# ka9q/ka9q-radio

Measured on NVIDIA H100. Metric: input Msamples/s through forward+filter+inverse at N channels, higher is better.
Workload: dtype f32

## Files before the change

### include/ka9q_gpu.h

```cpp
#ifndef KA9Q_GPU_H
#define KA9Q_GPU_H 1
#include <stddef.h>
#include <stdint.h>

#ifdef __cplusplus
extern "C" {
#endif

enum kgpu_type { KGPU_COMPLEX = 1, KGPU_REAL = 2 };
enum kgpu_format {
  KGPU_FMT_F32 = 0,
  KGPU_FMT_I16 = 1
};
enum kgpu_chan_flags {
  KGPU_CHAN_ISB = 1,
  KGPU_CHAN_BEAM = 4
};

typedef struct kgpu_master kgpu_master;
typedef struct kgpu_bank kgpu_bank;

struct kgpu_ingest_stats {
  unsigned long long energy;
  unsigned int clips;
// ... 118 lines not shown
int kgpu_bank_set_filter_on(kgpu_bank *b, int idx, double low, double high, double kaiser_beta, void *stream);
int kgpu_bank_set_response(kgpu_bank *b, int idx, float const *response);
int kgpu_bank_get_response(kgpu_bank *b, int idx, float *response);
int kgpu_bank_set_shift(kgpu_bank *b, int idx, int shift);
int kgpu_bank_set_flags(kgpu_bank *b, int idx, int flags);
int kgpu_bank_enable(kgpu_bank *b, int idx, int enabled);
int kgpu_bank_set_weights(kgpu_bank *b, int idx, double alpha_re, double alpha_im, double beta_re, double beta_im);
int kgpu_bank_set_osc(kgpu_bank *b, int idx, int enable, double phase_cycles, double freq_cps, double rate_cps2,
                      double block_adj_cycles);
int kgpu_bank_get_osc_phase(kgpu_bank *b, int idx, double *phase_cycles);
int kgpu_bank_set_block_counter(kgpu_bank *b, long counter);
long kgpu_bank_block_counter(kgpu_bank const *b);
int kgpu_bank_channels(kgpu_bank const *b);
long kgpu_bank_out_stride(kgpu_bank const *b);
long kgpu_bank_out_offset(kgpu_bank const *b, int idx);
int kgpu_bank_run(kgpu_bank *b, const void *d_spec, int nblocks, void *d_out, void *stream);
int kgpu_bank_run_ex(kgpu_bank *b, const void *d_spec, int nblocks, void *d_out, long out_pitch, float *d_power, void *stream);
int kgpu_bank_run_one(kgpu_bank *b, int idx, const void *d_spec, void *d_out, void *stream);
int kgpu_bank_run_one_ex(kgpu_bank *b, int idx, const void *d_spec, void *d_out, float *d_power , void *stream);
int kgpu_bank_noise(kgpu_bank *b, const void *d_spec, int nblocks, double samprate, double *d_n0, void *stream);

int kgpu_bank_fm_front(kgpu_bank *b, const void *d_out, long out_pitch, int nblocks, float *d_baseband, double *d_stats, void *stream);

int kgpu_bank_commit(kgpu_bank *b, void *stream);
int kgpu_use_static_kernels(int on);
int kgpu_use_cols_tma(int on);
int kgpu_cols_tma_fits(int L, int M, int in_type, int fmt, const void *d_in);
int kgpu_use_fused_forward(int on);
int kgpu_fused_forward_fits(int L, int M, int in_type, int fmt, const void *d_in);
int kgpu_fused_forward_options(int lead, int discard);
int kgpu_fused_shape(int *out);
int kgpu_fused_schedule(int nblocks, int lead, int ticket, int *out);
long kgpu_fused_discards(int blk, int idx, long *lines, long max);

int kgpu_plan_radices(int len, int *radices, int max);
int kgpu_plan_split(long n, int *n1, int *n2);
int kgpu_plan_radices_ex(int len, int *radices, int max);
int kgpu_plan_split_ex(long n, int *n1, int *n2);

int kgpu_multicast_copy(const void *d_src, void *mc_dst, unsigned long long bytes, int nctas, void *stream);

typedef struct kgpu_spectrum kgpu_spectrum;
kgpu_spectrum *kgpu_spectrum_create(int fft_n, int in_type, int bin_count);
int kgpu_spectrum_set_window(kgpu_spectrum *s, float const *window);
int kgpu_spectrum_run(kgpu_spectrum *s, const void *d_ring, long ring_samples, long end, int fmt, float scale,
                      const struct kgpu_scale_change *d_chg, int nchg, long long end_index, int derandomize, int shift, int fft_avg, double overlap, float *d_bins, void *stream);
int kgpu_spectrum_run_narrow(kgpu_spectrum *s, const void *d_ring, long ring_size, long ring_idx, int fft_avg,
                             double overlap, float *d_bins, int *fft_avg_used, void *stream);
int kgpu_spectrum_ring_append(void *d_ring, long ring_size, long ring_idx, const void *d_src, long olen, void *stream);
int kgpu_spectrum_describe(kgpu_spectrum const *s, char *buf, int buflen);
void kgpu_spectrum_destroy(kgpu_spectrum *s);
int kgpu_spectrum_plan(int fft_n, int in_type, char *buf, int buflen);

double kgpu_algorithmic_bytes(kgpu_master const *m, kgpu_bank const *b, int fmt);

#ifdef __cplusplus
}
#endif
#endif
```

### ka9q_radio_b200/capi.py

```python
from __future__ import annotations

import ctypes as C
import os
import subprocess
from pathlib import Path

PKG = Path(__file__).resolve().parent
LIB_PATH = PKG / "libka9qgpu.so"

KGPU_COMPLEX, KGPU_REAL = 1, 2
KGPU_FMT_F32, KGPU_FMT_I16 = 0, 1
KGPU_RAW_U8, KGPU_RAW_S8 = 1, 2
KGPU_RAW_S16, KGPU_RAW_U16, KGPU_RAW_SC16Q11 = 3, 4, 5
KGPU_RAW_F32, KGPU_RAW_CF32, KGPU_RAW_CF32_CNRMF, KGPU_RAW_CF32_FSCALE = 6, 7, 8, 9
KGPU_CHAN_ISB = 1
KGPU_CHAN_BEAM = 4

_lib = None


class KgpuError(RuntimeError):
    pass


# ... 63 lines not shown
    L.kgpu_siggen_destroy.argtypes = [vp]
    L.kgpu_siggen_generate.argtypes = [vp, ll, l, d, vp, i, vp, vp, i, l, l, vp]
    L.kgpu_siggen_state.argtypes = [vp, C.c_ulonglong, vp]
    L.kgpu_siggen_angles.argtypes = [vp, vp]
    L.filter_siggen_setup.argtypes = [vp, vp]
    L.write_genfilter.argtypes = [vp, i, d]
    L.filter_siggen_stats.argtypes = [vp, vp]
    L.kgpu_bank_define_ex.argtypes = [vp, i, i, i]
    L.kgpu_bank_define_wide.argtypes = [vp, i, i, i]
    L.kgpu_bank_define_huge.argtypes = [vp, i, i, i]
    L.kgpu_bank_define_ext.argtypes = [vp, i, i, i]
    L.kgpu_bank_define_any.argtypes = [vp, i, i, i]
    L.kgpu_chan_plan.argtypes = [i, i, C.c_char_p, i]
    L.kgpu_bank_set_weights.argtypes = [vp, i, d, d, d, d]
    L.kgpu_bank_set_osc.argtypes = [vp, i, i, d, d, d, d]
    L.kgpu_bank_get_osc_phase.argtypes = [vp, i, vp]
    L.kgpu_bank_set_block_counter.argtypes = [vp, l]
    L.kgpu_bank_block_counter.argtypes = [vp]
    L.kgpu_bank_block_counter.restype = l
    L.kgpu_bank_run_ex.argtypes = [vp, vp, i, vp, l, vp, vp]
    L.kgpu_bank_run_one_ex.argtypes = [vp, i, vp, vp, vp, vp]
    L.kgpu_bank_noise.argtypes = [vp, vp, i, d, vp, vp]
    L.kgpu_bank_fm_front.argtypes = [vp, vp, l, i, vp, vp, vp]
    L.kgpu_use_static_kernels.argtypes = [i]
    L.kgpu_use_cols_tma.argtypes = [i]
    L.kgpu_cols_tma_fits.argtypes = [i, i, i, i, vp]
    L.kgpu_use_fused_forward.argtypes = [i]
    L.kgpu_fused_forward_fits.argtypes = [i, i, i, i, vp]
    L.kgpu_fused_forward_options.argtypes = [i, i]
    L.kgpu_fused_shape.argtypes = [vp]
    L.kgpu_fused_schedule.argtypes = [i, i, i, vp]
    L.kgpu_fused_discards.argtypes = [i, i, vp, l]
    L.kgpu_fused_discards.restype = l
    L.kgpu_profile_enable.argtypes = [i]
    L.kgpu_profile_name.argtypes = [i]
    L.kgpu_profile_name.restype = C.c_char_p
    L.kgpu_profile_get.argtypes = [i, vp, vp]
    L.kgpu_plan_radices.argtypes = [i, vp, i]
    L.kgpu_plan_split.argtypes = [l, vp, vp]
    L.kgpu_plan_radices_ex.argtypes = [i, vp, i]
    L.kgpu_plan_split_ex.argtypes = [l, vp, vp]
    L.kgpu_multicast_copy.argtypes = [vp, vp, C.c_ulonglong, i, vp]
    L.kgpu_algorithmic_bytes.argtypes = [vp, vp, i]
    L.kgpu_algorithmic_bytes.restype = d
    L.kgpu_spectrum_create.restype = vp
    L.kgpu_spectrum_create.argtypes = [i, i, i]
    L.kgpu_spectrum_set_window.argtypes = [vp, vp]
    L.kgpu_spectrum_run.argtypes = [vp, vp, l, l, i, f, vp, i, C.c_longlong, i, i, i, d, vp, vp]
    L.kgpu_spectrum_run_narrow.argtypes = [vp, vp, l, l, i, d, vp, vp, vp]
    L.kgpu_spectrum_ring_append.argtypes = [vp, l, l, vp, l, vp]
    L.kgpu_spectrum_describe.argtypes = [vp, C.c_char_p, i]
    L.kgpu_spectrum_destroy.argtypes = [vp]
    L.kgpu_spectrum_plan.argtypes = [i, i, C.c_char_p, i]
    _lib = L
    return L


def exported_symbols() -> list[str]:
    import re

    hdr = (PKG.parent / "include" / "ka9q_gpu.h").read_text()
    hdr = re.sub(r"/\*.*?\*/", " ", hdr, flags=re.S)
    return sorted(set(re.findall(r"\b(kgpu_[a-z0-9_]+)\s*\(", hdr)))


def profile_snapshot() -> dict[str, tuple[float, int]]:
# ... 351 lines not shown
```

### ka9q_radio_b200/csrc/fwd_cols_r36.cuh

```cuda
#pragma once
#include <cuda.h>

#include "static_kernels_v2.cuh"

namespace kfft {

struct ColsR36Tables {
  float2 const *tw0;
  float2 const *twA;
  float2 const *twB;
};

__device__ __forceinline__ float2 r36_power(float2 const (&wb)[6], float2 const (&wa)[6], int t) {
  int const a = t / 6, b = t - 6 * a;
  if (a == 0) return wb[b];
  if (b == 0) return wa[a];
  return cmul(wa[a], wb[b]);
}

struct ColsR36Shape {
  static constexpr int BLK = 38, CP = 1378, T = 288;
  static constexpr size_t smem = sizeof(float2) * (size_t)(8 * CP + 360 + 80);
};

struct ColsR36Tma {
  static constexpr int BOX_ROWS = 216;
  static constexpr int F32_BOX_BYTES = BOX_ROWS * 64;
  static constexpr int I16_BOX_WORDS = 12, I16_BOX_BYTES = BOX_ROWS * I16_BOX_WORDS * 4;
  static constexpr int I16_ODD_OFF = 3 * I16_BOX_BYTES;
  static constexpr uint32_t bytes(int fmt) { return fmt == 0 ? 6 * F32_BOX_BYTES : 6 * I16_BOX_BYTES; }
};
static_assert(ColsR36Tma::bytes(0) + 112 <= sizeof(float2) * 8 * ColsR36Shape::CP &&
              ColsR36Tma::bytes(1) + 112 <= sizeof(float2) * 8 * ColsR36Shape::CP, "the raw tile lies in the float tile");
static_assert(ColsR36Tma::F32_BOX_BYTES % 128 == 0 && ColsR36Tma::I16_BOX_BYTES % 128 == 0, "box destinations 128-B aligned");

template <int FMT>
__device__ __forceinline__ float2 r36_ingest(int raw, int row, int col, int n2, Pass1Args const &a, unsigned long long &energy,
                                             unsigned int &clips) {
  int lo, hi;
  unpack_i16(raw, lo, hi);
  if (FMT == 2) {
    if (a.derandomize) {
      lo ^= (lo & 1) ? 0xfffffffe : 0;
      hi ^= (hi & 1) ? 0xfffffffe : 0;
    }
    if (a.stats && (long)row * n2 + col >= a.first_new) {
      energy += (unsigned long long)(lo * lo) + (unsigned long long)(hi * hi);
      clips += (lo > 32766 || lo < -32766) + (hi > 32766 || hi < -32766);
    }
  }
  return make_float2(i32_to_f32(lo), i32_to_f32(hi));
}

__device__ __forceinline__ void r36_stage0_store(float2 (&x)[36], float2 const *s_tw0, float2 *d, int ul) {
  constexpr int R = 36, BLK = ColsR36Shape::BLK;
  float2 wb[6], wa[6];
#pragma unroll
  for (int b = 1; b < 6; b++) {
    wb[b] = s_tw0[(b - 1) * 36 + ul];
    wa[b] = s_tw0[(4 + b) * 36 + ul];
  }
  d[0] = x[0];
#pragma unroll
  for (int t = 1; t < R; t++) d[t * BLK] = cmul(x[t], r36_power(wb, wa, t));
}

template <int FMT, int N2C, bool TMA, class Sync>
__device__ __forceinline__ void fwd_cols_r36_body(Pass1Args const &a, ColsR36Tables const &tb, CUtensorMap const *tmap,
                                                  unsigned char *smem_raw, uint64_t &tbar, int tid, int c0, int blk,
                                                  Sync const &sync) {
  constexpr int R = 36, BLK = ColsR36Shape::BLK, CP = ColsR36Shape::CP;
  float2 *tile = reinterpret_cast<float2 *>(smem_raw);
  float2 *s_tw0 = tile + 8 * CP;
  float2 *s_twB = s_tw0 + 360;
  int const c = tid & 7, ul = tid >> 3;
  int const n2 = N2C ? N2C : a.n2;
  int const ld = N2C ? (N2C + 15) / 16 * 16 : a.mid_ld;
  int const ncols = min(8, n2 - c0);
  bool const col_ok = c < ncols;
  int const n2g = c0 + c;
  float2 *mycol = tile + c * CP;
  unsigned char *const rtile = smem_raw + ((0u - smem_u32(smem_raw)) & 127u);
  if (tid == 0) {
    mbar_init(&tbar, 1);
    mbar_fence_init();
    if constexpr (TMA) {
      using T = ColsR36Tma;
      mbar_expect_tx(&tbar, 360 * 8 + 80 * 8 + T::bytes(FMT));
      if (FMT == 0) {
#pragma unroll
        for (int k = 0; k < 6; k++) tensor_g2s_3d(rtile + k * T::F32_BOX_BYTES, tmap, 2 * c0, k * T::BOX_ROWS, blk, &tbar);
      } else {
#pragma unroll
        for (int k = 0; k < 3; k++) {
          tensor_g2s_3d(rtile + k * T::I16_BOX_BYTES, tmap, c0, k * T::BOX_ROWS, blk, &tbar);
          tensor_g2s_3d(rtile + T::I16_ODD_OFF + k * T::I16_BOX_BYTES, tmap, n2 + c0 - (n2 & 2), k * T::BOX_ROWS, blk, &tbar);
        }
      }
    } else {
      mbar_expect_tx(&tbar, 360 * 8 + 80 * 8);
    }
    bulk_g2s(s_tw0, tb.tw0, 360 * 8, &tbar);
    bulk_g2s(s_twB, tb.twB + (long)c0 * 10, 80 * 8, &tbar);
  }
  sync();
  float2 const twA = col_ok ? ldg_stream_f2(tb.twA + (long)n2g * 36 + ul) : make_float2(1.f, 0.f);

  unsigned long long energy = 0;
  unsigned int clips = 0;
  if constexpr (TMA) {
    float2 x[R];
    mbar_wait(&tbar, 0);
    if (col_ok) {
      if (FMT == 0) {
        float2 const *src = reinterpret_cast<float2 const *>(rtile) + ul * 8 + c;
#pragma unroll
        for (int m = 0; m < R; m++) x[m] = src[R * 8 * m];
      } else {
        using T = ColsR36Tma;
        int const odd = ul & 1;
        int const *src = reinterpret_cast<int const *>(rtile + odd * T::I16_ODD_OFF) + (ul >> 1) * T::I16_BOX_WORDS + c +
                         odd * (n2 & 2);
#pragma unroll
        for (int m = 0; m < R; m++)
          x[m] = r36_ingest<FMT>(src[(R / 2) * T::I16_BOX_WORDS * m], ul + R * m, n2g, n2, a, energy, clips);
      }
      Dft<R, false>::run(x);
    }
    sync();
    if (col_ok) r36_stage0_store(x, s_tw0, mycol + ul, ul);
  } else if (col_ok) {
    float2 x[R];
    if (FMT == 0) {
      float2 const *src = reinterpret_cast<float2 const *>(a.in) + (long)blk * a.hop + n2g + (long)ul * n2;
#pragma unroll
      for (int m = 0; m < R; m++) x[m] = ldg_stream_f2(src + (long)(R * m) * n2);
    } else {
      int const *src = reinterpret_cast<int const *>(a.in) + (long)blk * a.hop + n2g + (long)ul * n2;
      int raw[R];
#pragma unroll
      for (int m = 0; m < R; m++) raw[m] = ldg_stream_b32(src + (long)(R * m) * n2);
#pragma unroll
      for (int m = 0; m < R; m++) x[m] = r36_ingest<FMT>(raw[m], ul + R * m, n2g, n2, a, energy, clips);
    }
    mbar_wait(&tbar, 0);
    Dft<R, false>::run(x);
    r36_stage0_store(x, s_tw0, mycol + ul, ul);
  } else {
    mbar_wait(&tbar, 0);
  }
  if (FMT == 2 && a.stats) {
#pragma unroll
    for (int o = 16; o > 0; o >>= 1) {
      energy += __shfl_xor_sync(0xffffffffu, energy, o);
      clips += __shfl_xor_sync(0xffffffffu, clips, o);
    }
    if ((tid & 31) == 0 && (energy | clips)) {
      atomicAdd(&a.stats[blk].energy, energy);
      atomicAdd(&a.stats[blk].clips, clips);
    }
  }
  sync();

  if (col_ok) {
    float2 x[R];
    float4 const *p4 = reinterpret_cast<float4 const *>(mycol + ul * BLK);
#pragma unroll
    for (int m = 0; m < R / 2; m++) {
      float4 const v = p4[m];
      x[2 * m] = make_float2(v.x, v.y);
      x[2 * m + 1] = make_float2(v.z, v.w);
    }
    Dft<R, false>::run(x);
    float2 wb[6], wa[6];
#pragma unroll
    for (int b = 1; b < 6; b++) {
      wb[b] = s_twB[c * 10 + (b - 1)];
      wa[b] = s_twB[c * 10 + (4 + b)];
    }
    float2 const w0 = make_float2(twA.x * a.out_scale, twA.y * a.out_scale);
    float2 *dst = a.mid + (long)blk * 1296 * ld + n2g + (long)ul * ld;
    dst[0] = cmul(x[0], w0);
#pragma unroll
    for (int k = 1; k < R; k++) dst[(long)(R * k) * ld] = cmul(x[k], cmul(w0, r36_power(wb, wa, k)));
  }
}

template <int FMT, int N2C>
__global__ void __launch_bounds__(ColsR36Shape::T, 2) fwd_cols_r36(Pass1Args const a, ColsR36Tables const tb) {
  extern __shared__ __align__(16) unsigned char smem_raw[];
  __shared__ __align__(8) uint64_t tbar;
  fwd_cols_r36_body<FMT, N2C, false>(a, tb, nullptr, smem_raw, tbar, threadIdx.x, blockIdx.x * 8, blockIdx.y,
                                     [] { __syncthreads(); });
}
template <int FMT, int N2C>
__global__ void __launch_bounds__(ColsR36Shape::T, 2)
    fwd_cols_r36_tma(Pass1Args const a, ColsR36Tables const tb, const __grid_constant__ CUtensorMap tmap) {
  extern __shared__ __align__(16) unsigned char smem_raw[];
  __shared__ __align__(8) uint64_t tbar;
  fwd_cols_r36_body<FMT, N2C, true>(a, tb, &tmap, smem_raw, tbar, threadIdx.x, blockIdx.x * 8, blockIdx.y,
                                    [] { __syncthreads(); });
}

}
```

### ka9q_radio_b200/csrc/fwd_fused.cuh

```cuda
#pragma once
#include "fwd_cols_r36.cuh"
#include "static_kernels_v2.cuh"

namespace kfft {

struct FusedShape {
  static constexpr int N1 = 1296, N2 = 1250;
  static constexpr int TILES = (N2 + 7) / 8;
  static constexpr int NC = (TILES + 1) / 2;
  static constexpr int NR = (N1 / 2 + 1 + RowsV2Shape<true>::IPC - 1) / RowsV2Shape<true>::IPC;
  static constexpr int T = 2 * ColsR36Shape::T;
  static constexpr int RT = RowsV2Shape<true>::T;
  static constexpr size_t smem = 2 * ColsR36Shape::smem > RowsV2Shape<true>::smem ? 2 * ColsR36Shape::smem : RowsV2Shape<true>::smem;
  static constexpr int DEFAULT_LEAD = 40;
  static_assert(ColsR36Shape::smem % 16 == 0, "the second tile's memory 16-byte aligned");
  static_assert(T % 32 == 0 && ColsR36Shape::T % 32 == 0 && RT % 32 == 0, "whole warps per tile and per R item");
};

enum FusedKind : int { kFusedCol = 0, kFusedRow = 1 };
struct FusedItem {
  int kind, blk, idx;
};

__host__ __device__ __forceinline__ FusedItem fused_item(int t, int nblocks, int lead) {
// ... 9 lines not shown
}

struct FusedArgs {
  unsigned *ctr;
  int nblocks, lead;
  int discard;
};

__device__ __forceinline__ void red_release_gpu_add(unsigned *p, unsigned v) {
  asm volatile("red.release.gpu.global.add.u32 [%0], %1;" ::"l"(p), "r"(v) : "memory");
}
__device__ __forceinline__ unsigned ld_acquire_gpu(unsigned const *p) {
  unsigned v;
  asm volatile("ld.acquire.gpu.global.u32 %0, [%1];" : "=r"(v) : "l"(p) : "memory");
  return v;
}

template <int FMT>
__global__ void __launch_bounds__(FusedShape::T, 1)
    fwd_fused_r36_v2(Pass1Args const a1, ColsR36Tables const t1, Pass2Args const a2, FwdTables const t2, FusedArgs const f,
                     const __grid_constant__ CUtensorMap tmap) {
  using F = FusedShape;
  extern __shared__ __align__(16) unsigned char smem_raw[];
  __shared__ __align__(8) uint64_t bars[RowsV2Shape<true>::COLS];
  __shared__ __align__(8) uint64_t tbar[2];
  __shared__ int s_ticket;
  int const tid = threadIdx.x;
  if (tid == 0) s_ticket = (int)atomicAdd(f.ctr, 1u);
  __syncthreads();
  FusedItem const it = fused_item(s_ticket, f.nblocks, f.lead);
  if (it.kind == kFusedCol) {
    int const h = tid >= ColsR36Shape::T, tile = 2 * it.idx + h;
    if (tile < F::TILES)
      fwd_cols_r36_body<FMT, F::N2, true>(a1, t1, &tmap, smem_raw + h * ColsR36Shape::smem, tbar[h], tid - h * ColsR36Shape::T,
                                           tile * 8, it.blk, [h] {
                                             asm volatile("bar.sync %0, %1;" ::"r"(1 + h), "n"(ColsR36Shape::T) : "memory");
                                           });
    __syncthreads();
    if (tid == 0) {
      __threadfence();
      red_release_gpu_add(f.ctr + 1 + fused_item(s_ticket, f.nblocks, f.lead).blk, 1u);
    }
    return;
  }
  if (tid >= F::RT) return;
  auto sync = [] { asm volatile("bar.sync 3, %0;" ::"n"(F::RT) : "memory"); };
  auto sync_or = [](int p) {
    int r;
    asm volatile("{\n\t.reg .pred q, o;\n\tsetp.ne.s32 q, %1, 0;\n\tbar.red.or.pred o, 3, %2, q;\n\tselp.s32 %0, 1, 0, o;\n\t}"
                 : "=r"(r)
                 : "r"(p), "n"(F::RT)
                 : "memory");
    return r;
  };
  if (tid == 0)
    while (ld_acquire_gpu(f.ctr + 1 + it.blk) < (unsigned)F::NC) __nanosleep(64);
  sync();
  fwd_rows_v2_body<true, F::N1, true, true>(a2, t2, smem_raw, bars, tbar[0], tid, it.blk, it.idx * RowsV2Shape<true>::IPC,
                                            sync, sync_or, f.discard);
}

}
```

### ka9q_radio_b200/csrc/kgpu.cu

```cuda
#include <cuda_runtime.h>
#include <cudaTypedefs.h>
#include <math.h>
#include <stdarg.h>
#include <stdio.h>
#include <stdlib.h>
#include <string.h>
#include <algorithm>
#include <complex>
#include <atomic>
#include <map>
#include <mutex>
#include <string>
#include <vector>

#include "../../include/ka9q_gpu.h"
#include "chan_kernels.cuh"
#include "chan_huge.cuh"
#include "chan_wide.cuh"
#include "fwd_kernels.cuh"
#include "noise_kernel.cuh"
#include "plan.cuh"
#include "static_kernels.cuh"
#include "static_kernels_v2.cuh"
#include "fwd_cols_r36.cuh"
#include "fwd_fused.cuh"
#include "fwd_2s.cuh"
#include "spectrum_kernels.cuh"
#include "bluestein_master.cuh"
#include "bluestein_chan.cuh"
#include "raw_ingest.cuh"
#include "iq_correct.cuh"
#include "siggen.cuh"

using namespace kfft;

static thread_local std::string g_err;
static std::atomic<unsigned long long> g_launches{0};

static std::atomic<int> g_static_on{1};
extern "C" int kgpu_use_static_kernels(int on) {
  g_static_on.store(on != 0);
  return 0;
}
static std::atomic<int> g_cols_tma{-1};
extern "C" int kgpu_use_cols_tma(int on) {
  g_cols_tma.store(on != 0);
  return 0;
}
static bool cols_tma_on() {
  int v = g_cols_tma.load();
  if (v < 0) {
    char const *e = getenv("KA9Q_COLS_TMA");
    g_cols_tma.compare_exchange_strong(v, (e && *e) ? (atoi(e) != 0) : 1);
    v = g_cols_tma.load();
  }
  return v != 0;
}
static std::atomic<int> g_fused{-1};
static std::atomic<int> g_fused_lead{FusedShape::DEFAULT_LEAD}, g_fused_discard{0};
extern "C" int kgpu_use_fused_forward(int on) {
  g_fused.store(on != 0);
  return 0;
}
static bool fused_on() {
  int v = g_fused.load();
  if (v < 0) {
    char const *e = getenv("KA9Q_FUSED_FWD");
    g_fused.compare_exchange_strong(v, (e && *e) ? (atoi(e) != 0) : 1);
    v = g_fused.load();
  }
  return v != 0;
}

static int fail(char const *fmt, ...) {
  char buf[512];
  va_list ap;
  va_start(ap, fmt);
  vsnprintf(buf, sizeof buf, fmt, ap);
  va_end(ap);
  g_err = buf;
  return -1;
}
#define CUDA_OK(expr)                                                                    \
  do {                                                                                   \
    cudaError_t e_ = (expr);                                                             \
    if (e_ != cudaSuccess) return fail("%s: %s (%s:%d)", #expr, cudaGetErrorString(e_), __FILE__, __LINE__); \
  } while (0)
#define CUDA_OKP(expr)                                                                   \
  do {                                                                                   \
    cudaError_t e_ = (expr);                                                             \
    if (e_ != cudaSuccess) {                                                             \
      fail("%s: %s (%s:%d)", #expr, cudaGetErrorString(e_), __FILE__, __LINE__);         \
      return nullptr;                                                                    \
    }                                                                                    \
  } while (0)

static int allow_smem(const void *func, size_t bytes) {
  if (bytes <= 48 * 1024) return 0;
  static std::mutex mu;
  static std::map<std::pair<int, const void *>, size_t> granted;
  int dev = 0;
  CUDA_OK(cudaGetDevice(&dev));
  std::lock_guard<std::mutex> lk(mu);
  size_t &g = granted[{dev, func}];
// ... 885 lines not shown
using ColsR36Fn = void (*)(Pass1Args, ColsR36Tables);
using ColsR36TmaFn = void (*)(Pass1Args, ColsR36Tables, CUtensorMap);
using Cols2sFn = void (*)(Pass1Args, Cols2sTables);
using RowsV2Fn = void (*)(Pass2Args, FwdTables);
using Cols2s = Cols2sShape<25, 32>;
using Rows2s = Rows2sShape<25, 25>;
static ColsR36Fn cols_r36_kernel(kgpu_master const *m, int f) {
  static ColsR36Fn const k[2][3] = {{fwd_cols_r36<0, 0>, fwd_cols_r36<1, 0>, fwd_cols_r36<2, 0>},
                                    {fwd_cols_r36<0, 1250>, fwd_cols_r36<1, 1250>, fwd_cols_r36<2, 1250>}};
  return k[m->n2c == 1250][f];
}
static ColsR36TmaFn cols_r36_tma_kernel(kgpu_master const *m, int f) {
  static ColsR36TmaFn const k[2][3] = {{fwd_cols_r36_tma<0, 0>, fwd_cols_r36_tma<1, 0>, fwd_cols_r36_tma<2, 0>},
                                       {fwd_cols_r36_tma<0, 1250>, fwd_cols_r36_tma<1, 1250>, fwd_cols_r36_tma<2, 1250>}};
  return k[m->n2c == 1250][f];
}
static Cols2sFn cols_2s_kernel(int f) {
  static Cols2sFn const k[3] = {fwd_cols_2s<0, 25, 32>, fwd_cols_2s<1, 25, 32>, fwd_cols_2s<2, 25, 32>};
  return k[f];
}
static RowsV2Fn rows_v2_kernel(kgpu_master const *m) {
  if (m->in_type == KGPU_REAL) return m->halved ? fwd_rows_v2<true, 1296, true> : fwd_rows_v2<true, 0, false>;
  return m->n1c ? fwd_rows_v2<false, 1296, false> : fwd_rows_v2<false, 0, false>;
}
static bool fused_pair(kgpu_master const *m) {
  return m->in_type == KGPU_REAL && m->cols == COLS_R36 && m->rows == ROWS_V2 && m->halved && m->n2c == FusedShape::N2 &&
         m->n1c == FusedShape::N1 && m->mid_ld % 16 == 0;
}
using FusedFn = void (*)(Pass1Args, ColsR36Tables, Pass2Args, FwdTables, FusedArgs, CUtensorMap);
static FusedFn fused_kernel(int f) {
  static FusedFn const k[3] = {fwd_fused_r36_v2<0>, fwd_fused_r36_v2<1>, fwd_fused_r36_v2<2>};
  return k[f];
}
static int rows_v2_threads(kgpu_master const *m) { return m->in_type == KGPU_REAL ? RowsV2Shape<true>::T : RowsV2Shape<false>::T; }
static size_t rows_v2_smem(kgpu_master const *m) {
  return m->in_type == KGPU_REAL ? RowsV2Shape<true>::smem : RowsV2Shape<false>::smem;
}

static int upload(float2 **d, std::vector<float2> const &v) {
  CUDA_OK(cudaMalloc(d, sizeof(float2) * v.size()));
  CUDA_OK(cudaMemcpy(*d, v.data(), sizeof(float2) * v.size(), cudaMemcpyHostToDevice));
  return 0;
}

static int bluestein_upload(Bluestein *b) {
  if (upload(&b->d_b, bluestein_bspec(b->n, b->P)) == 0) return 0;
  cudaFree(b->d_b);
  b->d_b = nullptr;
  return -1;
}

static void master_geometry(kgpu_master *m, int L, int M, int in_type) {
  m->L = L;
  m->M = M;
  m->N = L + M - 1;
  m->in_type = in_type;
  m->bins = (in_type == KGPU_COMPLEX) ? m->N : m->N / 2 + 1;
  m->nc = (in_type == KGPU_COMPLEX) ? m->N : m->N / 2;
  m->spec_stride = ((long)m->bins + 3) / 4 * 4;
}

static void master_shape(kgpu_master *m, int L, int M, int in_type, Split2 const &sp, bool ext) {
  master_geometry(m, L, M, in_type);
  m->sp = sp;
  m->ext = ext;
  m->pitch1 = column_pitch(sp.n1);
// ... 48 lines not shown
    std::vector<float2> t0(360), tA((size_t)n2 * 36), tB((size_t)(n2 + 8) * 10, make_float2(0.f, 0.f));
    for (int e = 0; e < 10; e++)
      for (int j = 0; j < 36; j++) t0[(size_t)e * 36 + j] = root((long)j * kPow[e], 1296);
    for (long c = 0; c < n2; c++) {
      for (int t = 0; t < 36; t++) tA[(size_t)c * 36 + t] = root(c * t, m->nc);
      for (int e = 0; e < 10; e++) tB[(size_t)c * 10 + e] = root(c * 36 * kPow[e], m->nc);
    }
    if (upload(&m->d_tw0, t0) || upload(&m->d_twA, tA) || upload(&m->d_twB, tB)) return -1;
    for (int f = 0; f < 3; f++)
      if (allow_smem((const void *)cols_r36_kernel(m, f), ColsR36Shape::smem) ||
          allow_smem((const void *)cols_r36_tma_kernel(m, f), ColsR36Shape::smem))
        return -1;
  }
  if (m->cols == COLS_2S) {
    constexpr int RA = 25, RB = 32, RC = 25, RD = 25;
    std::vector<float2> t0((size_t)Cols2s::TW0, make_float2(0.f, 0.f)), tA((size_t)n2 * RA),
        tB((size_t)(n2 + 8) * Cols2s::NP1, make_float2(0.f, 0.f)), r0((size_t)Rows2s::TW0, make_float2(0.f, 0.f));
    for (int e = 0; e < Cols2s::NP0; e++)
      for (int j = 0; j < RB; j++) t0[(size_t)e * RB + j] = root((long)j * Pow<RA>::exponent(e), n1);
    for (long c = 0; c < n2; c++) {
      for (int t = 0; t < RA; t++) tA[(size_t)c * RA + t] = root(c * t, m->nc);
      for (int e = 0; e < Cols2s::NP1; e++) tB[(size_t)c * Cols2s::NP1 + e] = root(c * RA * Pow<RB>::exponent(e), m->nc);
    }
    for (int e = 0; e < Rows2s::NP0; e++)
      for (int j = 0; j < RD; j++) r0[(size_t)e * RD + j] = root((long)j * Pow<RC>::exponent(e), n2);
    if (upload(&m->d_tw0, t0) || upload(&m->d_twA, tA) || upload(&m->d_twB, tB) || upload(&m->d_rtw0, r0)) return -1;
    for (int f = 0; f < 3; f++)
      if (allow_smem((const void *)cols_2s_kernel(f), Cols2s::smem)) return -1;
    if (allow_smem((const void *)fwd_rows_2s<25, 25>, Rows2s::smem)) return -1;
  }
  if (m->rows == ROWS_V2 && allow_smem((const void *)rows_v2_kernel(m), rows_v2_smem(m))) return -1;
  if (fused_pair(m))
    for (int f = 0; f < 3; f++)
      if (allow_smem((const void *)fused_kernel(f), FusedShape::smem)) return -1;
  if (m->ext) {
    if (allow_smem((const void *)fwd_cols_ext<0>, m->smem1) || allow_smem((const void *)fwd_cols_ext<1>, m->smem1) ||
        allow_smem((const void *)fwd_rows_ext, m->smem2))
      return -1;
  } else if (allow_smem((const void *)fwd_cols_kernel<0>, m->smem1) || allow_smem((const void *)fwd_cols_kernel<1>, m->smem1) ||
             allow_smem((const void *)fwd_rows_kernel, m->smem2)) {
    return -1;
  }
  return 0;
}

extern "C" void kgpu_master_destroy(kgpu_master *m) {
  if (!m) return;
  if (m->ext) {
    free_tile_plan(m->xplan1);
    free_tile_plan(m->xplan2);
  }
  cudaFree(m->d_rootD);
  cudaFree(m->d_rootC);
  cudaFree(m->d_tw0);
  cudaFree(m->d_twA);
  cudaFree(m->d_twB);
  cudaFree(m->d_rtw0);
  cudaFree(m->mid.p);
  cudaFree(m->fused_ctr.p);
  cudaFree(m->d_notch);
  kgpu_master_destroy(m->bs);
  cudaFree(m->blue.d_b);
  cudaFree(m->b_in.p);
  cudaFree(m->b_out.p);
  delete m;
}
extern "C" int kgpu_master_points(kgpu_master const *m) { return m ? m->N : -1; }
// ... 180 lines not shown
  return fused_fits(&m, d_in, fmt) ? 1 : 0;
}

extern "C" int kgpu_fused_forward_options(int lead, int discard) {
  if (lead < 0 || lead > FusedShape::NC) return fail("kgpu_fused_forward_options: lead %d outside 0..%d", lead, FusedShape::NC);
  g_fused_lead.store(lead);
  g_fused_discard.store(discard != 0);
  return 0;
}

extern "C" int kgpu_fused_shape(int *out) {
  if (!out) return fail("kgpu_fused_shape: bad arguments");
  out[0] = FusedShape::NC;
  out[1] = FusedShape::NR;
  out[2] = FusedShape::N1;
  out[3] = (FusedShape::N2 + 15) / 16 * 16;
  out[4] = FusedShape::DEFAULT_LEAD;
  return 0;
}

extern "C" int kgpu_fused_schedule(int nblocks, int lead, int ticket, int *out) {
  if (nblocks < 1 || lead < 0 || lead > FusedShape::NC || ticket < 0 || ticket >= nblocks * (FusedShape::NC + FusedShape::NR) ||
      !out)
    return fail("kgpu_fused_schedule: bad arguments");
  FusedItem const it = fused_item(ticket, nblocks, lead);
  out[0] = it.kind;
  out[1] = it.blk;
  out[2] = it.idx;
  out[3] = it.kind == kFusedRow ? it.blk : -1;
  out[4] = it.kind == kFusedRow ? FusedShape::NC : 0;
  return 0;
}

extern "C" long kgpu_fused_discards(int blk, int idx, long *lines, long max) {
  using S = RowsV2Shape<true>;
  if (blk < 0 || idx < 0 || idx >= FusedShape::NR || max < 0) return fail("kgpu_fused_discards: bad arguments");
  int const ld = (FusedShape::N2 + 15) / 16 * 16;
  long n = 0;
  for (int col = 0; col < S::COLS; col++) {
    RowItem const it = row_item(idx * S::IPC + (col >> 1), FusedShape::N1, true);
    int const row = (col & 1) == 0 ? (it.kind != kRowEmpty ? it.row_a : -1) : (it.kind == kRowPair ? it.row_b : -1);
    if (row < 0) continue;
    for (int l = 0; l < mid_row_lines(ld); l++, n++)
      if (lines && n < max) lines[n] = mid_line(blk, FusedShape::N1, row, ld, l);
  }
  return n;
}

static int cols_tma_map(kgpu_master const *m, void const *d_in, int fmt, int nblocks, CUtensorMap *map) {
  static PFN_cuTensorMapEncodeTiled const encode = [] {
    void *fn = nullptr;
    cudaDriverEntryPointQueryResult q;
    if (cudaGetDriverEntryPoint("cuTensorMapEncodeTiled", &fn, cudaEnableDefault, &q) != cudaSuccess ||
        q != cudaDriverEntryPointSuccess)
      fn = nullptr;
    return (PFN_cuTensorMapEncodeTiled)fn;
  }();
  if (!encode) return fail("kgpu_forward: the driver has no cuTensorMapEncodeTiled");
  bool const i16 = fmt == KGPU_FMT_I16;
  cuuint64_t const n1 = (cuuint64_t)m->sp.n1, n2 = (cuuint64_t)m->sp.n2;
  cuuint64_t const hop = (cuuint64_t)(m->in_type == KGPU_REAL ? m->L / 2 : m->L);
  cuuint64_t const dim[3] = {2 * n2, i16 ? n1 / 2 : n1, (cuuint64_t)nblocks};
  cuuint64_t const stride[2] = {8 * n2, hop * (i16 ? 4 : 8)};
  cuuint32_t const box[3] = {(cuuint32_t)(i16 ? ColsR36Tma::I16_BOX_WORDS : 16), ColsR36Tma::BOX_ROWS, 1};
  cuuint32_t const unit[3] = {1, 1, 1};
  CUresult const r = encode(map, i16 ? CU_TENSOR_MAP_DATA_TYPE_UINT32 : CU_TENSOR_MAP_DATA_TYPE_FLOAT32, 3, const_cast<void *>(d_in),
                            dim, stride, box, unit, CU_TENSOR_MAP_INTERLEAVE_NONE, CU_TENSOR_MAP_SWIZZLE_NONE,
                            CU_TENSOR_MAP_L2_PROMOTION_L2_128B, CU_TENSOR_MAP_FLOAT_OOB_FILL_NONE);
  if (r != CUDA_SUCCESS) return fail("kgpu_forward: cuTensorMapEncodeTiled failed (%d)", (int)r);
  return 0;
}

static Pass2Args rows_args(kgpu_master const *m, Pass1Args const &a1, void *d_spec) {
  Pass2Args a2;
  a2.mid = a1.mid;
  a2.n1 = m->sp.n1;
  a2.n2 = m->sp.n2;
  a2.nc = m->nc;
  a2.plan = m->plan2;
  a2.pitch = m->pitch2;
  a2.real_split = (m->in_type == KGPU_REAL);
  a2.rootD = m->d_rootD;
  a2.spec = (float2 *)d_spec;
  a2.spec_stride = m->spec_stride;
  a2.mid_ld = a1.mid_ld;
  return a2;
}

static int fused_span(kgpu_master *m, const void *d_in, int fmt, int f, int nblocks, void *d_spec, cudaStream_t st,
                      Pass1Args const &a1) {
  using F = FusedShape;
  size_t const ctr_bytes = sizeof(unsigned) * (size_t)(1 + nblocks);
  if (grow(m->fused_ctr, ctr_bytes, st, "kgpu_forward")) return -1;
  CUtensorMap map;
  if (cols_tma_map(m, d_in, fmt, nblocks, &map)) return -1;
  FusedArgs fa;
  fa.ctr = (unsigned *)m->fused_ctr.p;
  fa.nblocks = nblocks;
  fa.lead = g_fused_lead.load();
  fa.discard = g_fused_discard.load();
  CUDA_OK(cudaMemsetAsync(fa.ctr, 0, ctr_bytes, st));
  {
    ProfScope ps(K_FWD_FUSED, st);
    fused_kernel(f)<<<(unsigned)(nblocks * (F::NC + F::NR)), F::T, F::smem, st>>>(a1, ColsR36Tables{m->d_tw0, m->d_twA, m->d_twB},
                                                                       rows_args(m, a1, d_spec), FwdTables{m->d_rootC}, fa, map);
  }
  g_launches++;
  CUDA_OK(cudaGetLastError());
  return 0;
}

static int forward_span(kgpu_master *m, const void *d_in, int fmt, float scale, int derandomize, int nblocks, void *d_spec,
                        void *d_stats, cudaStream_t st, float2 *mid) {
  bool const use_static = g_static_on.load() != 0;
  ColsKernel const cols = use_static ? m->cols : COLS_GENERIC;
  RowsKernel const rows = use_static ? m->rows : ROWS_GENERIC;
  Pass1Args a1;
  a1.in = d_in;
  a1.hop = (m->in_type == KGPU_REAL) ? m->L / 2 : m->L;
  a1.n1 = m->sp.n1;
  a1.n2 = m->sp.n2;
  a1.nc = m->nc;
  a1.plan = m->plan1;
  a1.pitch = m->pitch1;
  a1.scale = scale;
  a1.derandomize = derandomize;
  a1.first_new = (m->in_type == KGPU_REAL) ? (m->M - 1) / 2 : (m->M - 1);
  a1.mid = mid;
  a1.stats = (fmt == KGPU_FMT_I16) ? (IngestStats *)d_stats : nullptr;
  a1.out_scale = (fmt == KGPU_FMT_I16 ? scale : 1.0f) * (m->halved ? 0.5f : 1.0f);
  a1.mid_ld = use_static ? m->mid_ld : m->sp.n2;
  int const f = (fmt != KGPU_FMT_I16) ? 0 : ((derandomize || a1.stats) ? 2 : 1);
  if (nblocks >= 2 && use_static && cols_tma_on() && fused_on() && fused_fits(m, d_in, fmt)) return fused_span(m, d_in, fmt, f, nblocks, d_spec, st, a1);
  dim3 const g1((unsigned)((m->sp.n2 + kTile - 1) / kTile), (unsigned)nblocks);
  {
    ProfScope ps(K_FWD_COLS, st);
    switch (cols) {
      case COLS_2S:
        cols_2s_kernel(f)<<<g1, Cols2s::T, Cols2s::smem, st>>>(a1, Cols2sTables{m->d_tw0, m->d_twA, m->d_twB});
        break;
      case COLS_R36:
        if (cols_tma_on() && cols_tma_fits(m, d_in, fmt)) {
          CUtensorMap map;
          if (cols_tma_map(m, d_in, fmt, nblocks, &map)) return -1;
          cols_r36_tma_kernel(m, f)<<<g1, ColsR36Shape::T, ColsR36Shape::smem, st>>>(a1, ColsR36Tables{m->d_tw0, m->d_twA, m->d_twB}, map);
        } else {
          cols_r36_kernel(m, f)<<<g1, ColsR36Shape::T, ColsR36Shape::smem, st>>>(a1, ColsR36Tables{m->d_tw0, m->d_twA, m->d_twB});
        }
        break;
      case COLS_GENERIC:
        if (m->ext && f) fwd_cols_ext<1><<<g1, kFwdThreads, m->smem1, st>>>(a1, m->xplan1);
        else if (m->ext) fwd_cols_ext<0><<<g1, kFwdThreads, m->smem1, st>>>(a1, m->xplan1);
        else if (f) fwd_cols_kernel<1><<<g1, kFwdThreads, m->smem1, st>>>(a1);
        else fwd_cols_kernel<0><<<g1, kFwdThreads, m->smem1, st>>>(a1);
        break;
    }
  }
  g_launches++;
  Pass2Args const a2 = rows_args(m, a1, d_spec);
  dim3 const g2((unsigned)(rows == ROWS_GENERIC ? m->n_item_ctas : m->n_rows_ctas), (unsigned)nblocks);
  {
    ProfScope ps(K_FWD_ROWS, st);
    switch (rows) {
      case ROWS_2S:
        fwd_rows_2s<25, 25><<<g2, Rows2s::T, Rows2s::smem, st>>>(a2, m->d_rtw0);
        break;
// ... 1353 lines not shown
```

Measured before the change: 103,600.

## Add persistent warp-specialized fused forward kernel and L2 evict-last mid stores

Adds an opt-in persistent fused forward kernel (mode 3) that splits each CTA into a row-pass engine and a 4-column column-pass engine. The two engines pull work tickets from global counters and synchronize per block through release/acquire counters. The column tile geometry is templated on column count. Separately, the existing fused kernel now writes the intermediate mid buffer with an L2 evict_last cache hint so the rows pass can re-read it from L2. The new kernel runs only via env/setting, and the hint may displace other L2 data.

```diff
diff --git a/include/ka9q_gpu.h b/include/ka9q_gpu.h
--- a/include/ka9q_gpu.h
+++ b/include/ka9q_gpu.h
@@ -174,6 +174,8 @@
 int kgpu_fused_shape(int *out);
 int kgpu_fused_schedule(int nblocks, int lead, int ticket, int *out);
 long kgpu_fused_discards(int blk, int idx, long *lines, long max);
+int kgpu_fused2_shape(int *out);
+int kgpu_fused2_schedule(int nblocks, int queue, int ticket, int *out);
 
 int kgpu_plan_radices(int len, int *radices, int max);
 int kgpu_plan_split(long n, int *n1, int *n2);
diff --git a/ka9q_radio_b200/capi.py b/ka9q_radio_b200/capi.py
--- a/ka9q_radio_b200/capi.py
+++ b/ka9q_radio_b200/capi.py
@@ -119,6 +119,8 @@
     L.kgpu_fused_schedule.argtypes = [i, i, i, vp]
     L.kgpu_fused_discards.argtypes = [i, i, vp, l]
     L.kgpu_fused_discards.restype = l
+    L.kgpu_fused2_shape.argtypes = [vp]
+    L.kgpu_fused2_schedule.argtypes = [i, i, i, vp]
     L.kgpu_profile_enable.argtypes = [i]
     L.kgpu_profile_name.argtypes = [i]
     L.kgpu_profile_name.restype = C.c_char_p
diff --git a/ka9q_radio_b200/csrc/fwd_cols_r36.cuh b/ka9q_radio_b200/csrc/fwd_cols_r36.cuh
--- a/ka9q_radio_b200/csrc/fwd_cols_r36.cuh
+++ b/ka9q_radio_b200/csrc/fwd_cols_r36.cuh
@@ -18,21 +18,28 @@
   return cmul(wa[a], wb[b]);
 }
 
-struct ColsR36Shape {
-  static constexpr int BLK = 38, CP = 1378, T = 288;
-  static constexpr size_t smem = sizeof(float2) * (size_t)(8 * CP + 360 + 80);
+template <int NCOL>
+struct ColsR36Geom {
+  static_assert(NCOL == 8 || NCOL == 4, "8- or 4-column tiles");
+  static constexpr int BLK = 38, CP = NCOL == 8 ? 1378 : 1380, T = (36 * NCOL + 31) / 32 * 32;
+  static constexpr int LOG = NCOL == 8 ? 3 : 2;
+  static constexpr size_t smem = sizeof(float2) * (size_t)(NCOL * CP + 360 + 10 * NCOL);
 };
-
-struct ColsR36Tma {
+using ColsR36Shape = ColsR36Geom<8>;
+
+template <int NCOL>
+struct ColsR36TmaT {
   static constexpr int BOX_ROWS = 216;
-  static constexpr int F32_BOX_BYTES = BOX_ROWS * 64;
-  static constexpr int I16_BOX_WORDS = 12, I16_BOX_BYTES = BOX_ROWS * I16_BOX_WORDS * 4;
+  static constexpr int F32_BOX_FLOATS = 2 * NCOL, F32_BOX_BYTES = BOX_ROWS * F32_BOX_FLOATS * 4;
+  static constexpr int I16_BOX_WORDS = NCOL + 4, I16_BOX_BYTES = BOX_ROWS * I16_BOX_WORDS * 4;
   static constexpr int I16_ODD_OFF = 3 * I16_BOX_BYTES;
   static constexpr uint32_t bytes(int fmt) { return fmt == 0 ? 6 * F32_BOX_BYTES : 6 * I16_BOX_BYTES; }
+  static_assert(bytes(0) + 112 <= sizeof(float2) * NCOL * ColsR36Geom<NCOL>::CP &&
+                bytes(1) + 112 <= sizeof(float2) * NCOL * ColsR36Geom<NCOL>::CP, "the raw tile lies in the float tile");
+  static_assert(F32_BOX_BYTES % 128 == 0 && I16_BOX_BYTES % 128 == 0, "box destinations 128-B aligned");
+  static_assert(F32_BOX_FLOATS * 4 % 16 == 0 && I16_BOX_WORDS * 4 % 16 == 0, "box widths whole 16-byte units");
 };
-static_assert(ColsR36Tma::bytes(0) + 112 <= sizeof(float2) * 8 * ColsR36Shape::CP &&
-              ColsR36Tma::bytes(1) + 112 <= sizeof(float2) * 8 * ColsR36Shape::CP, "the raw tile lies in the float tile");
-static_assert(ColsR36Tma::F32_BOX_BYTES % 128 == 0 && ColsR36Tma::I16_BOX_BYTES % 128 == 0, "box destinations 128-B aligned");
+using ColsR36Tma = ColsR36TmaT<8>;
 
 template <int FMT>
 __device__ __forceinline__ float2 r36_ingest(int raw, int row, int col, int n2, Pass1Args const &a, unsigned long long &energy,
@@ -65,19 +72,20 @@
   for (int t = 1; t < R; t++) d[t * BLK] = cmul(x[t], r36_power(wb, wa, t));
 }
 
-template <int FMT, int N2C, bool TMA, class Sync>
+template <int FMT, int N2C, bool TMA, int NCOL = 8, bool KEEP_MID = false, class Sync>
 __device__ __forceinline__ void fwd_cols_r36_body(Pass1Args const &a, ColsR36Tables const &tb, CUtensorMap const *tmap,
                                                   unsigned char *smem_raw, uint64_t &tbar, int tid, int c0, int blk,
                                                   Sync const &sync) {
-  constexpr int R = 36, BLK = ColsR36Shape::BLK, CP = ColsR36Shape::CP;
+  using G = ColsR36Geom<NCOL>;
+  constexpr int R = 36, BLK = G::BLK, CP = G::CP;
   float2 *tile = reinterpret_cast<float2 *>(smem_raw);
-  float2 *s_tw0 = tile + 8 * CP;
+  float2 *s_tw0 = tile + NCOL * CP;
   float2 *s_twB = s_tw0 + 360;
-  int const c = tid & 7, ul = tid >> 3;
+  int const c = tid & (NCOL - 1), ul = tid >> G::LOG;
   int const n2 = N2C ? N2C : a.n2;
   int const ld = N2C ? (N2C + 15) / 16 * 16 : a.mid_ld;
-  int const ncols = min(8, n2 - c0);
-  bool const col_ok = c < ncols;
+  int const ncols = min(NCOL, n2 - c0);
+  bool const col_ok = c < ncols && (G::T == R * NCOL || ul < R);
   int const n2g = c0 + c;
   float2 *mycol = tile + c * CP;
   unsigned char *const rtile = smem_raw + ((0u - smem_u32(smem_raw)) & 127u);
@@ -85,8 +93,8 @@
     mbar_init(&tbar, 1);
     mbar_fence_init();
     if constexpr (TMA) {
-      using T = ColsR36Tma;
-      mbar_expect_tx(&tbar, 360 * 8 + 80 * 8 + T::bytes(FMT));
+      using T = ColsR36TmaT<NCOL>;
+      mbar_expect_tx(&tbar, 360 * 8 + NCOL * 80 + T::bytes(FMT));
       if (FMT == 0) {
 #pragma unroll
         for (int k = 0; k < 6; k++) tensor_g2s_3d(rtile + k * T::F32_BOX_BYTES, tmap, 2 * c0, k * T::BOX_ROWS, blk, &tbar);
@@ -98,10 +106,10 @@
         }
       }
     } else {
-      mbar_expect_tx(&tbar, 360 * 8 + 80 * 8);
+      mbar_expect_tx(&tbar, 360 * 8 + NCOL * 80);
     }
     bulk_g2s(s_tw0, tb.tw0, 360 * 8, &tbar);
-    bulk_g2s(s_twB, tb.twB + (long)c0 * 10, 80 * 8, &tbar);
+    bulk_g2s(s_twB, tb.twB + (long)c0 * 10, NCOL * 80, &tbar);
   }
   sync();
   float2 const twA = col_ok ? ldg_stream_f2(tb.twA + (long)n2g * 36 + ul) : make_float2(1.f, 0.f);
@@ -113,11 +121,11 @@
     mbar_wait(&tbar, 0);
     if (col_ok) {
       if (FMT == 0) {
-        float2 const *src = reinterpret_cast<float2 const *>(rtile) + ul * 8 + c;
-#pragma unroll
-        for (int m = 0; m < R; m++) x[m] = src[R * 8 * m];
+        float2 const *src = reinterpret_cast<float2 const *>(rtile) + ul * NCOL + c;
+#pragma unroll
+        for (int m = 0; m < R; m++) x[m] = src[R * NCOL * m];
       } else {
-        using T = ColsR36Tma;
+        using T = ColsR36TmaT<NCOL>;
         int const odd = ul & 1;
         int const *src = reinterpret_cast<int const *>(rtile + odd * T::I16_ODD_OFF) + (ul >> 1) * T::I16_BOX_WORDS + c +
                          odd * (n2 & 2);
@@ -180,9 +188,20 @@
     }
     float2 const w0 = make_float2(twA.x * a.out_scale, twA.y * a.out_scale);
     float2 *dst = a.mid + (long)blk * 1296 * ld + n2g + (long)ul * ld;
-    dst[0] = cmul(x[0], w0);
-#pragma unroll
-    for (int k = 1; k < R; k++) dst[(long)(R * k) * ld] = cmul(x[k], cmul(w0, r36_power(wb, wa, k)));
+    if constexpr (KEEP_MID) {
+      uint64_t pol;
+      asm("createpolicy.fractional.L2::evict_last.b64 %0, 1.0;" : "=l"(pol));
+      auto st = [pol](float2 *p, float2 v) {
+        asm volatile("st.global.L2::cache_hint.v2.f32 [%0], {%1, %2}, %3;" ::"l"(p), "f"(v.x), "f"(v.y), "l"(pol) : "memory");
+      };
+      st(dst, cmul(x[0], w0));
+#pragma unroll
+      for (int k = 1; k < R; k++) st(dst + (long)(R * k) * ld, cmul(x[k], cmul(w0, r36_power(wb, wa, k))));
+    } else {
+      dst[0] = cmul(x[0], w0);
+#pragma unroll
+      for (int k = 1; k < R; k++) dst[(long)(R * k) * ld] = cmul(x[k], cmul(w0, r36_power(wb, wa, k)));
+    }
   }
 }
 
diff --git a/ka9q_radio_b200/csrc/fwd_fused.cuh b/ka9q_radio_b200/csrc/fwd_fused.cuh
--- a/ka9q_radio_b200/csrc/fwd_fused.cuh
+++ b/ka9q_radio_b200/csrc/fwd_fused.cuh
@@ -65,7 +65,7 @@
   if (it.kind == kFusedCol) {
     int const h = tid >= ColsR36Shape::T, tile = 2 * it.idx + h;
     if (tile < F::TILES)
-      fwd_cols_r36_body<FMT, F::N2, true>(a1, t1, &tmap, smem_raw + h * ColsR36Shape::smem, tbar[h], tid - h * ColsR36Shape::T,
+      fwd_cols_r36_body<FMT, F::N2, true, 8, true>(a1, t1, &tmap, smem_raw + h * ColsR36Shape::smem, tbar[h], tid - h * ColsR36Shape::T,
                                            tile * 8, it.blk, [h] {
                                              asm volatile("bar.sync %0, %1;" ::"r"(1 + h), "n"(ColsR36Shape::T) : "memory");
                                            });
diff --git a/ka9q_radio_b200/csrc/fwd_fused2.cuh b/ka9q_radio_b200/csrc/fwd_fused2.cuh
--- /dev/null
+++ b/ka9q_radio_b200/csrc/fwd_fused2.cuh
@@ -0,0 +1,122 @@
+#pragma once
+#include "fwd_fused.cuh"
+
+namespace kfft {
+
+struct Fused2Shape {
+  static constexpr int N1 = 1296, N2 = 1250, NCOL = 4;
+  using CG = ColsR36Geom<NCOL>;
+  static constexpr int NT = (N2 + NCOL - 1) / NCOL;
+  static constexpr int NR = FusedShape::NR;
+  static constexpr int LAG = 2;
+  static constexpr int RT = RowsV2Shape<true>::T;
+  static constexpr int CT = CG::T;
+  static constexpr int T = RT + CT;
+  static constexpr size_t row_smem = RowsV2Shape<true>::smem;
+  static constexpr size_t smem = row_smem + CG::smem;
+  static_assert(row_smem % 16 == 0, "the column engine's memory 16-byte aligned");
+  static_assert(T % 32 == 0 && CT % 32 == 0 && RT % 32 == 0, "whole warps per engine");
+  static_assert(smem + 256 <= 227 * 1024, "both engines' shared memory in one SM");
+};
+
+enum Fused2Queue : int { kFused2Col = 0, kFused2Row = 1 };
+struct Fused2Item {
+  int blk, idx;
+  int wait, need;
+};
+__host__ __device__ __forceinline__ Fused2Item fused2_item(int queue, int t, int nblocks) {
+  using F = Fused2Shape;
+  if (queue == kFused2Col) {
+    int const b = t / F::NT;
+    return b >= F::LAG ? Fused2Item{b, t - b * F::NT, 2 + nblocks + b - F::LAG, F::NR} : Fused2Item{b, t - b * F::NT, -1, 0};
+  }
+  int const b = t / F::NR;
+  return {b, t - b * F::NR, 2 + b, F::NT};
+}
+
+struct Fused2Args {
+  unsigned *ctr;
+  int nblocks;
+};
+
+__device__ __forceinline__ void fence_proxy_async_smem() { asm volatile("fence.proxy.async.shared::cta;" ::: "memory"); }
+__device__ __forceinline__ void mbar_inval(uint64_t *bar) {
+  asm volatile("mbarrier.inval.shared::cta.b64 [%0];" ::"r"(smem_u32(bar)) : "memory");
+}
+__device__ __forceinline__ void fused2_wait(unsigned const *ctr, Fused2Item const &it) {
+  if (it.wait >= 0)
+    while (ld_acquire_gpu(ctr + it.wait) < (unsigned)it.need) __nanosleep(64);
+}
+
+template <int FMT>
+__global__ void __launch_bounds__(Fused2Shape::T, 1)
+    fwd_fused_r36_v3(Pass1Args const a1, ColsR36Tables const t1, Pass2Args const a2, FwdTables const t2, Fused2Args const f,
+                     const __grid_constant__ CUtensorMap tmap) {
+  using F = Fused2Shape;
+  extern __shared__ __align__(16) unsigned char smem_raw[];
+  __shared__ __align__(8) uint64_t bars[RowsV2Shape<true>::COLS];
+  __shared__ __align__(8) uint64_t tbar[2];
+  __shared__ int s_ticket[2];
+  int const tid = threadIdx.x;
+  if (tid < F::RT) {
+    auto sync = [] { asm volatile("bar.sync 3, %0;" ::"n"(F::RT) : "memory"); };
+    auto sync_or = [](int p) {
+      int r;
+      asm volatile("{\n\t.reg .pred q, o;\n\tsetp.ne.s32 q, %1, 0;\n\tbar.red.or.pred o, 3, %2, q;\n\tselp.s32 %0, 1, 0, o;\n\t}"
+                   : "=r"(r)
+                   : "r"(p), "n"(F::RT)
+                   : "memory");
+      return r;
+    };
+    int const total = f.nblocks * F::NR;
+    for (;;) {
+      if (tid == 0) {
+        int const t = (int)atomicAdd(f.ctr + 1, 1u);
+        s_ticket[0] = t;
+        if (t < total) fused2_wait(f.ctr, fused2_item(kFused2Row, t, f.nblocks));
+      }
+      sync();
+      int const t = s_ticket[0];
+      if (t >= total) return;
+      Fused2Item const it = fused2_item(kFused2Row, t, f.nblocks);
+      fwd_rows_v2_body<true, F::N1, true, true>(a2, t2, smem_raw, bars, tbar[0], tid, it.blk, it.idx * RowsV2Shape<true>::IPC,
+                                                sync, sync_or, false);
+      fence_proxy_async_smem();
+      sync();
+      if ((tid & 31) == 0) {
+        mbar_inval(&bars[tid >> 5]);
+        if (tid == 0) {
+          mbar_inval(&tbar[0]);
+          __threadfence();
+          red_release_gpu_add(f.ctr + 2 + f.nblocks + it.blk, 1u);
+        }
+      }
+    }
+  } else {
+    int const ct = tid - F::RT;
+    auto sync = [] { asm volatile("bar.sync 4, %0;" ::"n"(F::CT) : "memory"); };
+    unsigned char *const smem = smem_raw + F::row_smem;
+    int const total = f.nblocks * F::NT;
+    for (;;) {
+      if (ct == 0) {
+        int const t = (int)atomicAdd(f.ctr, 1u);
+        s_ticket[1] = t;
+        if (t < total) fused2_wait(f.ctr, fused2_item(kFused2Col, t, f.nblocks));
+      }
+      sync();
+      int const t = s_ticket[1];
+      if (t >= total) return;
+      Fused2Item const it = fused2_item(kFused2Col, t, f.nblocks);
+      fwd_cols_r36_body<FMT, F::N2, true, F::NCOL, true>(a1, t1, &tmap, smem, tbar[1], ct, it.idx * F::NCOL, it.blk, sync);
+      fence_proxy_async_smem();
+      sync();
+      if (ct == 0) {
+        mbar_inval(&tbar[1]);
+        __threadfence();
+        red_release_gpu_add(f.ctr + 2 + it.blk, 1u);
+      }
+    }
+  }
+}
+
+}
diff --git a/ka9q_radio_b200/csrc/kgpu.cu b/ka9q_radio_b200/csrc/kgpu.cu
--- a/ka9q_radio_b200/csrc/kgpu.cu
+++ b/ka9q_radio_b200/csrc/kgpu.cu
@@ -24,6 +24,7 @@
 #include "static_kernels_v2.cuh"
 #include "fwd_cols_r36.cuh"
 #include "fwd_fused.cuh"
+#include "fwd_fused2.cuh"
 #include "fwd_2s.cuh"
 #include "spectrum_kernels.cuh"
 #include "bluestein_master.cuh"
@@ -56,20 +57,22 @@
   }
   return v != 0;
 }
+enum FusedMode { kFusedOff = 0, kFusedDefault = 1, kFusedV2 = 2, kFusedV3 = 3 };
 static std::atomic<int> g_fused{-1};
 static std::atomic<int> g_fused_lead{FusedShape::DEFAULT_LEAD}, g_fused_discard{0};
+static int fused_mode_of(int on) { return on >= kFusedOff && on <= kFusedV3 ? on : kFusedDefault; }
 extern "C" int kgpu_use_fused_forward(int on) {
-  g_fused.store(on != 0);
-  return 0;
-}
-static bool fused_on() {
+  g_fused.store(fused_mode_of(on));
+  return 0;
+}
+static int fused_mode() {
   int v = g_fused.load();
   if (v < 0) {
     char const *e = getenv("KA9Q_FUSED_FWD");
-    g_fused.compare_exchange_strong(v, (e && *e) ? (atoi(e) != 0) : 1);
+    g_fused.compare_exchange_strong(v, (e && *e) ? fused_mode_of(atoi(e)) : kFusedDefault);
     v = g_fused.load();
   }
-  return v != 0;
+  return v == kFusedDefault ? kFusedV2 : v;
 }
 
 static int fail(char const *fmt, ...) {
@@ -1021,6 +1024,11 @@
   static FusedFn const k[3] = {fwd_fused_r36_v2<0>, fwd_fused_r36_v2<1>, fwd_fused_r36_v2<2>};
   return k[f];
 }
+using Fused2Fn = void (*)(Pass1Args, ColsR36Tables, Pass2Args, FwdTables, Fused2Args, CUtensorMap);
+static Fused2Fn fused2_kernel(int f) {
+  static Fused2Fn const k[3] = {fwd_fused_r36_v3<0>, fwd_fused_r36_v3<1>, fwd_fused_r36_v3<2>};
+  return k[f];
+}
 static int rows_v2_threads(kgpu_master const *m) { return m->in_type == KGPU_REAL ? RowsV2Shape<true>::T : RowsV2Shape<false>::T; }
 static size_t rows_v2_smem(kgpu_master const *m) {
   return m->in_type == KGPU_REAL ? RowsV2Shape<true>::smem : RowsV2Shape<false>::smem;
@@ -1135,7 +1143,8 @@
   if (m->rows == ROWS_V2 && allow_smem((const void *)rows_v2_kernel(m), rows_v2_smem(m))) return -1;
   if (fused_pair(m))
     for (int f = 0; f < 3; f++)
-      if (allow_smem((const void *)fused_kernel(f), FusedShape::smem)) return -1;
+      if (allow_smem((const void *)fused_kernel(f), FusedShape::smem) || allow_smem((const void *)fused2_kernel(f), Fused2Shape::smem))
+        return -1;
   if (m->ext) {
     if (allow_smem((const void *)fwd_cols_ext<0>, m->smem1) || allow_smem((const void *)fwd_cols_ext<1>, m->smem1) ||
         allow_smem((const void *)fwd_rows_ext, m->smem2))
@@ -1382,6 +1391,27 @@
   return 0;
 }
 
+extern "C" int kgpu_fused2_shape(int *out) {
+  if (!out) return fail("kgpu_fused2_shape: bad arguments");
+  out[0] = Fused2Shape::NT;
+  out[1] = Fused2Shape::NR;
+  out[2] = Fused2Shape::LAG;
+  out[3] = Fused2Shape::NCOL;
+  return 0;
+}
+
+extern "C" int kgpu_fused2_schedule(int nblocks, int queue, int ticket, int *out) {
+  int const per = queue == kFused2Col ? Fused2Shape::NT : Fused2Shape::NR;
+  if (nblocks < 1 || (queue != kFused2Col && queue != kFused2Row) || ticket < 0 || ticket >= nblocks * per || !out)
+    return fail("kgpu_fused2_schedule: bad arguments");
+  Fused2Item const it = fused2_item(queue, ticket, nblocks);
+  out[0] = it.blk;
+  out[1] = it.idx;
+  out[2] = it.wait;
+  out[3] = it.need;
+  return 0;
+}
+
 extern "C" long kgpu_fused_discards(int blk, int idx, long *lines, long max) {
   using S = RowsV2Shape<true>;
   if (blk < 0 || idx < 0 || idx >= FusedShape::NR || max < 0) return fail("kgpu_fused_discards: bad arguments");
@@ -1397,7 +1427,9 @@
   return n;
 }
 
+template <int NCOL = 8>
 static int cols_tma_map(kgpu_master const *m, void const *d_in, int fmt, int nblocks, CUtensorMap *map) {
+  using T = ColsR36TmaT<NCOL>;
   static PFN_cuTensorMapEncodeTiled const encode = [] {
     void *fn = nullptr;
     cudaDriverEntryPointQueryResult q;
@@ -1412,7 +1444,9 @@
   cuuint64_t const hop = (cuuint64_t)(m->in_type == KGPU_REAL ? m->L / 2 : m->L);
   cuuint64_t const dim[3] = {2 * n2, i16 ? n1 / 2 : n1, (cuuint64_t)nblocks};
   cuuint64_t const stride[2] = {8 * n2, hop * (i16 ? 4 : 8)};
-  cuuint32_t const box[3] = {(cuuint32_t)(i16 ? ColsR36Tma::I16_BOX_WORDS : 16), ColsR36Tma::BOX_ROWS, 1};
+  cuuint32_t const box[3] = {(cuuint32_t)(i16 ? T::I16_BOX_WORDS : T::F32_BOX_FLOATS), T::BOX_ROWS, 1};
+  if (NCOL * 4 % 16 != 0 || (i16 && (n2 - (n2 & 2)) % 4 != 0))
+    return fail("kgpu_forward: %d-column tensor boxes would start off 16-byte alignment", NCOL);
   cuuint32_t const unit[3] = {1, 1, 1};
   CUresult const r = encode(map, i16 ? CU_TENSOR_MAP_DATA_TYPE_UINT32 : CU_TENSOR_MAP_DATA_TYPE_FLOAT32, 3, const_cast<void *>(d_in),
                             dim, stride, box, unit, CU_TENSOR_MAP_INTERLEAVE_NONE, CU_TENSOR_MAP_SWIZZLE_NONE,
@@ -1454,6 +1488,30 @@
     ProfScope ps(K_FWD_FUSED, st);
     fused_kernel(f)<<<(unsigned)(nblocks * (F::NC + F::NR)), F::T, F::smem, st>>>(a1, ColsR36Tables{m->d_tw0, m->d_twA, m->d_twB},
                                                                        rows_args(m, a1, d_spec), FwdTables{m->d_rootC}, fa, map);
+  }
+  g_launches++;
+  CUDA_OK(cudaGetLastError());
+  return 0;
+}
+
+static int fused2_span(kgpu_master *m, const void *d_in, int fmt, int f, int nblocks, void *d_spec, cudaStream_t st,
+                       Pass1Args const &a1) {
+  using F = Fused2Shape;
+  size_t const ctr_bytes = sizeof(unsigned) * (size_t)(2 + 2 * nblocks);
+  if (grow(m->fused_ctr, ctr_bytes, st, "kgpu_forward")) return -1;
+  CUtensorMap map;
+  if (cols_tma_map<F::NCOL>(m, d_in, fmt, nblocks, &map)) return -1;
+  int dev = 0, sms = 0;
+  CUDA_OK(cudaGetDevice(&dev));
+  CUDA_OK(cudaDeviceGetAttribute(&sms, cudaDevAttrMultiProcessorCount, dev));
+  Fused2Args fa;
+  fa.ctr = (unsigned *)m->fused_ctr.p;
+  fa.nblocks = nblocks;
+  CUDA_OK(cudaMemsetAsync(fa.ctr, 0, ctr_bytes, st));
+  {
+    ProfScope ps(K_FWD_FUSED, st);
+    fused2_kernel(f)<<<(unsigned)sms, F::T, F::smem, st>>>(a1, ColsR36Tables{m->d_tw0, m->d_twA, m->d_twB}, rows_args(m, a1, d_spec),
+                                                           FwdTables{m->d_rootC}, fa, map);
   }
   g_launches++;
   CUDA_OK(cudaGetLastError());
@@ -1481,7 +1539,9 @@
   a1.out_scale = (fmt == KGPU_FMT_I16 ? scale : 1.0f) * (m->halved ? 0.5f : 1.0f);
   a1.mid_ld = use_static ? m->mid_ld : m->sp.n2;
   int const f = (fmt != KGPU_FMT_I16) ? 0 : ((derandomize || a1.stats) ? 2 : 1);
-  if (nblocks >= 2 && use_static && cols_tma_on() && fused_on() && fused_fits(m, d_in, fmt)) return fused_span(m, d_in, fmt, f, nblocks, d_spec, st, a1);
+  if (nblocks >= 2 && use_static && cols_tma_on() && fused_mode() != kFusedOff && fused_fits(m, d_in, fmt))
+    return fused_mode() == kFusedV2 ? fused_span(m, d_in, fmt, f, nblocks, d_spec, st, a1)
+                                    : fused2_span(m, d_in, fmt, f, nblocks, d_spec, st, a1);
   dim3 const g1((unsigned)((m->sp.n2 + kTile - 1) / kTile), (unsigned)nblocks);
   {
     ProfScope ps(K_FWD_COLS, st);
```

New measurement: 105,600 (median of 6 runs). 1.02x the previous value.
